# wjwei-handsome/wgatools

Hardware: AMD Instinct MI355X
Metric: paf_cigar_ops_per_s (paf2maf+stat) (higher is better)
Workload: dtype u8

## Files before the change

### wgatools_amd/csrc/capi_paf2maf.inc

```
static inline u32 job_tiles_for(int param, u64 nt) {
  if (param >= 1) return param > (int)WGA_S_MAX_JOB_TILES ? WGA_S_MAX_JOB_TILES : (u32)param;
  return nt < 200000ull ? 4u : 8u;
}

struct PrepassWs {
  u64 nt, jobs;
  u32 job_tiles;
  size_t rec_bytes, desc_bytes, list_bytes, flag_bytes, skip_bytes, zero_bytes, total;
  wga_rec_desc* recs = nullptr;
  wga_tile_desc* tdesc = nullptr;
  u32 *wide_list = nullptr, *fast_list = nullptr, *counts = nullptr;
  u8* tile_flag = nullptr;
  u32* job_skip = nullptr;
  PrepassWs(u32 n, u64 nt_, u32 job_tiles_, bool stream) : nt(nt_), jobs((nt_ + job_tiles_ - 1) / job_tiles_), job_tiles(job_tiles_) {
    rec_bytes = ((size_t)n * sizeof(wga_rec_desc) + 255) & ~(size_t)255;
    desc_bytes = (size_t)nt * sizeof(wga_tile_desc);
    list_bytes = 2 * (size_t)nt * sizeof(u32);
    flag_bytes = stream ? (((size_t)nt + 255) & ~(size_t)255) : 0;
    skip_bytes = stream ? (((size_t)jobs * sizeof(u32) + 255) & ~(size_t)255) : 0;
    zero_bytes = 256 + flag_bytes + skip_bytes;
    total = rec_bytes + desc_bytes + list_bytes + zero_bytes;
  }
  void carve(void* base) {
    char* const p = (char*)base;
    recs = (wga_rec_desc*)p;
    tdesc = (wga_tile_desc*)(p + rec_bytes);
    wide_list = (u32*)(p + rec_bytes + desc_bytes);
    fast_list = wide_list + nt;
    counts = (u32*)(p + rec_bytes + desc_bytes + list_bytes);
    tile_flag = flag_bytes ? (u8*)counts + 256 : nullptr;
    job_skip = flag_bytes ? (u32*)(tile_flag + flag_bytes) : nullptr;
  }
};
static int launch_tile_base(wga_ctx* c, const wga_cigar_batch* b, const PrepassWs& w, const wga_tile_sum* tiles, int mode,
                            int force_slow) {
  WGA_LAUNCH(k_tile_base, (u32)((w.nt + 255) / 256), WGA_BLOCK, c->stream, (const u64*)b->d_op_off, (u64)b->n_ops, tiles,
             (const wga_rec_desc*)w.recs, w.tdesc, mode, (const u8*)w.tile_flag, w.job_tiles, force_slow, w.job_skip, w.counts,
             w.fast_list, w.wide_list);
  LAUNCH_CHECK();
  return WGA_OK;
}

extern "C" {

size_t wga_tile_ws_bytes(uint64_t n_ops) { return (size_t)(n_tiles(n_ops) * sizeof(wga_tile_sum)) + 16; }

int wga_cigar_stat(wga_ctx* c, const wga_cigar_batch* b, wga_cigar_counts* d_counts,
                   wga_rec_diag* d_diag, void* d_tile_ws) {
  int rc = ctx_bind(c);
  if (rc) return rc;
  if ((rc = check_batch(b))) return rc;
  if (b->n == 0) return WGA_OK;
  if (!d_counts || !d_diag) return fail(WGA_E_INVALID_ARG, "d_counts / d_diag null", nullptr);
  RT_CHECK(rt_memset(d_counts, 0, (size_t)b->n * sizeof(wga_cigar_counts), c->stream));
  RT_CHECK(rt_memset(d_diag, 0xFF, (size_t)b->n * sizeof(wga_rec_diag), c->stream));
  u64 nt = n_tiles(b->n_ops);
  if (nt == 0) return WGA_OK;
  void* ws;
  if ((rc = ctx_scratch(c, (size_t)nt * sizeof(wga_tile_rec), &ws))) return rc;
  wga_tile_rec* tile_rec = (wga_tile_rec*)ws;
  WGA_LAUNCH(k_tile_rec, (u32)((nt + 255) / 256), WGA_BLOCK, c->stream, (const u64*)b->d_op_off,
             b->d_strand_neg, b->n, (u64)b->n_ops, tile_rec);
  LAUNCH_CHECK();
  const u32 grid = (u32)((nt + 3) / 4);
  WGA_LAUNCH(k_cigar_stat, grid, WGA_BLOCK, c->stream, b->d_ops, (const u64*)b->d_op_off,
             b->d_strand_neg, b->n, (u64)b->n_ops, (const wga_tile_rec*)tile_rec, d_counts, d_diag,
             (wga_tile_sum*)d_tile_ws);
  LAUNCH_CHECK();
  return WGA_OK;
}

int wga_exclusive_scan_u64(wga_ctx* c, uint32_t n, const uint64_t* d_in, uint64_t* d_out) {
  int rc = ctx_bind(c);
  if (rc) return rc;
  if (!d_out || (n && !d_in)) return fail(WGA_E_INVALID_ARG, "null array", nullptr);
  ScanPlain f;
  f.in = (const u64*)d_in;
  return run_scan(c, f, n, (u64*)d_out);
}

int wga_paf2maf_layout(wga_ctx* c, uint32_t n, const wga_cigar_counts* d_counts,
                       const uint64_t* d_t_src_len, const uint64_t* d_q_src_len,
                       const uint32_t* d_pre_t, const uint32_t* d_pre_q, const uint32_t* d_post,
                       uint64_t* d_t_row_off, uint64_t* d_q_row_off, uint64_t* d_rec_off) {
  int rc = ctx_bind(c);
  if (rc) return rc;
  if (!d_rec_off) return fail(WGA_E_INVALID_ARG, "d_rec_off null", nullptr);
  if (n && (!d_counts || !d_t_src_len || !d_q_src_len || !d_t_row_off || !d_q_row_off))
    return fail(WGA_E_INVALID_ARG, "null array", nullptr);
  ScanLayout f;
  f.counts = d_counts;
  f.t_src_len = (const u64*)d_t_src_len;
  f.q_src_len = (const u64*)d_q_src_len;
  f.pre_t = d_pre_t;
  f.pre_q = d_pre_q;
  f.post = d_post;
  rc = run_scan(c, f, n, (u64*)d_rec_off);
  if (rc) return rc;
  if (n) {
    WGA_LAUNCH(k_layout_rows, (n + 255u) / 256u, WGA_BLOCK, c->stream, f, n, (const u64*)d_rec_off,
               (u64*)d_t_row_off, (u64*)d_q_row_off);
    LAUNCH_CHECK();
  }
  return WGA_OK;
}

int wga_paf2maf_expand(wga_ctx* c, const wga_cigar_batch* b, const wga_cigar_counts* d_counts,
                       const void* d_tile_ws, const uint8_t* d_t_fa, uint64_t t_fa_bytes,
                       const uint64_t* d_t_src_off, const uint64_t* d_t_src_len,
                       const uint8_t* d_q_fa, uint64_t q_fa_bytes, const uint64_t* d_q_src_off,
                       const uint64_t* d_q_src_len, uint8_t* d_out, const uint64_t* d_t_row_off,
                       const uint64_t* d_q_row_off, wga_rec_diag* d_diag) {
  int rc = ctx_bind(c);
  if (rc) return rc;
  if ((rc = check_batch(b))) return rc;
  if (b->n == 0 || b->n_ops == 0) return WGA_OK;
  if (!d_counts || !d_tile_ws || !d_t_src_off || !d_t_src_len || !d_q_src_off || !d_q_src_len ||
      !d_out || !d_t_row_off || !d_q_row_off || !d_diag)
    return fail(WGA_E_INVALID_ARG, "null array", nullptr);
  if ((t_fa_bytes && !d_t_fa) || (q_fa_bytes && !d_q_fa)) return fail(WGA_E_INVALID_ARG, "null sequence pool", nullptr);
  u64 nt = n_tiles(b->n_ops);
  if (nt > 0x7FFFFFFFull) return fail(WGA_E_INVALID_ARG, "batch too large for one launch", nullptr);
  const int variant = c->expand_variant >= 0 ? c->expand_variant : WGA_AUTO_LONG_VARIANT;
  c->expand_variant_used = variant;
  const bool stream = variant == 3;
  PrepassWs w(b->n, nt, job_tiles_for(c->expand_job_tiles, nt), stream);
  void* ws;
  if ((rc = ctx_scratch(c, w.total, &ws))) return rc;
  w.carve(ws);
  if (stream) RT_CHECK(rt_memset(w.counts, 0, w.zero_bytes, c->stream));
  WGA_LAUNCH(k_rec_desc, (b->n + 255u) / 256u, WGA_BLOCK, c->stream, b->n, d_counts,
             b->d_strand_neg, (const u64*)d_t_src_off, (const u64*)d_t_src_len,
             (const u64*)d_q_src_off, (const u64*)d_q_src_len, (const u64*)d_t_row_off,
             (const u64*)d_q_row_off, w.recs, (const u64*)b->d_op_off, (u64)t_fa_bytes, (u64)q_fa_bytes, w.tile_flag);
  LAUNCH_CHECK();
  if ((rc = launch_tile_base(c, b, w, (const wga_tile_sum*)d_tile_ws, 0, c->expand_force_slow))) return rc;
  if (stream) c->stream_counts = w.counts;
  ExpandArgs a;
  a.ops = b->d_ops;
  a.op_off = (const u64*)b->d_op_off;
  a.n_ops = b->n_ops;
  a.tdesc = w.tdesc;
  a.recs = w.recs;
  a.t_fa = d_t_fa;
  a.t_fa_bytes = t_fa_bytes;
  a.q_fa = d_q_fa;
  a.q_fa_bytes = q_fa_bytes;
  a.out = d_out;
  a.diag = d_diag;
  a.force_slow = c->expand_force_slow;
  a.no_table = c->expand_no_table;
  a.drain_min = c->expand_drain_min ? c->expand_drain_min : ((u64)t_fa_bytes + (u64)q_fa_bytes > WGA_DRAIN_POOL_BYTES ? 16u : 32u);
  a.tile_count = nullptr;
  a.tile_list = nullptr;
  a.n_rec = b->n;
  a.job_tiles = w.job_tiles;
  a.job_skip = w.job_skip;
  c->expand_drain_min_used = a.drain_min;
  const uint32_t slot = c->ev_n % (uint32_t)wga_ctx::kTimingRing;
  if (c->timing) RT_CHECK(rt_event_record(c->ev[2 * slot], c->stream));
  if (stream) {
    WGA_LAUNCH(k_paf2maf_expand_s, (u32)w.jobs, 128u, c->stream, a);
    LAUNCH_CHECK();
    const u32 side_grid = nt < 256 ? (u32)nt : 256u;
    a.tile_count = w.counts;
    a.tile_list = w.fast_list;
    WGA_LAUNCH(k_paf2maf_expand_list, side_grid, WGA_BLOCK, c->stream, a);
    LAUNCH_CHECK();
    a.force_slow = 1;
    a.tile_count = w.counts + 1;
    a.tile_list = w.wide_list;
    WGA_LAUNCH(k_paf2maf_expand_list, side_grid, WGA_BLOCK, c->stream, a);
    LAUNCH_CHECK();
  } else {
    WGA_LAUNCH(k_paf2maf_expand, (u32)nt, WGA_BLOCK, c->stream, a);
    LAUNCH_CHECK();
  }
  if (c->timing) {
    RT_CHECK(rt_event_record(c->ev[2 * slot + 1], c->stream));
    c->ev_n++;
  }
  return WGA_OK;
}

int wga_ctx_expand_timing(wga_ctx* c, double* ms_sum, uint32_t* launches) {
  int rc = ctx_bind(c);
  if (rc) return rc;
  if (!ms_sum || !launches) return fail(WGA_E_INVALID_ARG, "null argument", nullptr);
  *ms_sum = 0.0;
  *launches = 0;
  if (!c->timing) return WGA_OK;
  const uint32_t n = c->ev_n < (uint32_t)wga_ctx::kTimingRing ? c->ev_n : (uint32_t)wga_ctx::kTimingRing;
  for (uint32_t k = 0; k < n; k++) {
    float ms = 0.0f;
    RT_CHECK(rt_event_elapsed_ms(c->ev[2 * k], c->ev[2 * k + 1], &ms));
    *ms_sum += (double)ms;
  }
  *launches = n;
  c->ev_n = 0;
  return WGA_OK;
}

int wga_scatter_bytes(wga_ctx* c, uint32_t n, const uint8_t* d_src, const uint64_t* d_src_off,
                      uint8_t* d_dst, const uint64_t* d_dst_off) {
  int rc = ctx_bind(c);
  if (rc) return rc;
  if (n == 0) return WGA_OK;
  if (!d_src || !d_src_off || !d_dst || !d_dst_off) return fail(WGA_E_INVALID_ARG, "null array", nullptr);
  WGA_LAUNCH(k_scatter_bytes, (n + 3u) / 4u, WGA_BLOCK, c->stream, n, d_src, (const u64*)d_src_off,
             d_dst, (const u64*)d_dst_off);
  LAUNCH_CHECK();
  return WGA_OK;
}

int wga_counts_total(wga_ctx* c, uint32_t n, const wga_cigar_counts* d_counts, uint64_t* d_totals) {
  int rc = ctx_bind(c);
  if (rc) return rc;
  if (!d_totals || (n && !d_counts)) return fail(WGA_E_INVALID_ARG, "null array", nullptr);
  static_assert(sizeof(wga_cigar_counts) == 88, "wga_cigar_counts is 11 u64");
  RT_CHECK(rt_memset(d_totals, 0, 88, c->stream));
  if (n == 0) return WGA_OK;
  u32 grid = (u32)(((u64)n * 11ull + 253ull * 8ull - 1ull) / (253ull * 8ull));
  if (grid > 2048u) grid = 2048u;
  WGA_LAUNCH(k_counts_total, grid, WGA_BLOCK, c->stream, n, (const u64*)d_counts, (u64*)d_totals);
  LAUNCH_CHECK();
  return WGA_OK;
}

}
```

### wgatools_amd/csrc/wga_capi.cpp

```cpp
#include <stdio.h>
#include <stdlib.h>
#include <string.h>

#include <algorithm>
#include <string>
#include <utility>
#include <vector>

#include <type_traits>

#include "wga_kernels.h"
#include "wga_k1_stat.h"
#include "wga_scan.h"
#include "wga_k2_v1.h"
#include "wga_kernels_k2s.h"
#include "wga_k_class.h"
#include "wga_k_peers.h"
#include "wga_k5_pafcov.h"
#include "wga_k6_pafpseudo.h"
#include "wga_k3_maf.h"
#include "wga_k7_paf_call.h"
#include "wga_k8_tokenise.h"
#include "wga_text_out.h"
#include "wga_chain_items.h"
#include "wga_paf_head.h"
#include "wga_k9_bed.h"
#include "wga_k10_chain.h"
#include "wga_k11_bridges.h"
#include "wga_k12_dotplot.h"
#include "wga_k13_splitters.h"
#include "wga_k15_fasta.h"
#include "wga_k18_bgzf_deflate.h"
#include "wga_k16_paf_call_vcf.h"
#include "wga_k17_bgzf_inflate.h"
#include "wga_k19_maf_call.h"
#include "wga_k20_maf_chunk.h"
#include "wga_k21_maf_slice.h"
#include "wga_k22_maf_rewrite.h"
#include "wga_k23_chain_split.h"
#include "wga_k24_paf_filter.h"
#include "wga_k25_chain_write.h"
#include "wga_k26_dotplot_csv.h"
#include "wga_k27_chain2paf.h"
#include "wga_k28_maf2paf.h"
#include "wga_k29_paf_fix.h"
#include "wga_k30_chain_heads.h"
#include "wga_k31_pseudo_frame.h"
#include "wga_k32_maf_frame.h"
#include "wga_k33_stat_rows.h"

struct DevBuf {
  void* mem = nullptr;
  size_t cap = 0;
  int reserve(wga_ctx* c, size_t need, size_t grow, bool* grew = nullptr);
  void release() {
    if (mem) (void)rt_free(mem);
    mem = nullptr, cap = 0;
  }
};

struct CallKey {
  int who = 0;
  struct Arr {
    const void* p = nullptr;
    size_t bytes = 0;
  } arr[5];
  uint64_t par[6] = {0, 0, 0, 0, 0, 0};
  bool operator==(const CallKey& o) const {
    bool same = who == o.who;
    for (int k = 0; k < 5; k++) same = same && arr[k].p == o.arr[k].p && arr[k].bytes == o.arr[k].bytes;
    for (int k = 0; k < 6; k++) same = same && par[k] == o.par[k];
    return same;
  }
};
struct CallCache {
  CallKey key;
  bool valid = false;
  bool take(const CallKey& k, bool is_fill) {
    const bool hit = is_fill && valid && key == k;
    valid = false;
    return hit;
  }
  void keep(const CallKey& k) { key = k, valid = true; }
  void written(const void* lo, size_t bytes) {
    const uintptr_t a = (uintptr_t)lo, z = a + (bytes ? bytes : 1);
    for (const CallKey::Arr& q : key.arr)
      if (q.p && (uintptr_t)q.p < z && (uintptr_t)q.p + (q.bytes ? q.bytes : 1) > a) valid = false;
  }
};

struct wga_ctx {
  int device = 0;
  wga_stream_t own_stream = nullptr;
  wga_stream_t stream = nullptr;
  int expand_force_slow = 0;
  int expand_no_table = 0;
  unsigned expand_drain_min = 0;
  unsigned expand_drain_min_used = 0;
  uint64_t op_long_ops = 16384;
  uint64_t op_piece_ops = 8192;
  uint64_t maf_long_cols = 32768;
  uint64_t maf_piece_cols = 16384;
  unsigned paf_pair_hash_bits = 64;
  unsigned maf_group = 0;
  DevBuf maf_tab;
  bool maf_hdr_clean = false;
  CallCache maf_cache;
  int expand_variant = -1;
  int expand_variant_used = 0;
  int expand_job_tiles = 0;
  int pseudo_variant = 3;
  const u32* pseudo_counts = nullptr;
  const u32* stream_counts = nullptr;
  DevBuf scratch;
  struct OpTab {
    DevBuf buf;
    CallCache cache;
    uint32_t np = 0;
    bool all = false;
    u64* piece_off = nullptr;
    u32* piece_rec = nullptr;
    void* pieces = nullptr;
  } op_tab;
  struct ClassTab {
    DevBuf buf;
    CallCache cache;
    wga_tile_sum* tiles = nullptr;
    wga_class_sums* rec_sums = nullptr;
  } class_tab;
  struct ElemScan {
    DevBuf buf;
    CallCache cache;
  } elem_scan;
  struct Cov {
    DevBuf pieces;
    DevBuf tile_list;
    DevBuf order;
    std::vector<u64> order_key;
    DevBuf list;
    u64 list_rcap = 0;
  } cov;
  bool rs_have_ev = false;
  rt_event_t rs_ready, rs_done;
  std::vector<wga_stream_t> rs_streams;
  std::vector<rt_event_t> rs_copied;
  bool rs_same_device_ok = false;
  bool rs_staged = false;
#ifdef WGA_EMU
  u32 cov_spin_limit = 64;
#else
  u32 cov_spin_limit = 1u << 12;
#endif
  static const int kTimingRing = 64;
  bool timing = false;
  rt_event_t ev[2 * kTimingRing];
  uint32_t ev_n = 0;
};

static thread_local std::string g_last_error;

static int fail(int code, const char* what, const char* detail) {
  g_last_error = std::string(what) + (detail ? std::string(": ") + detail : std::string());
  return code;
}
#define RT_CHECK(expr)                                      \
  do {                                                      \
    const char* _e = (expr);                                \
    if (_e) return fail(WGA_E_HIP, #expr, _e);              \
  } while (0)
#define LAUNCH_CHECK()                                      \
  do {                                                      \
    const char* _e = rt_launch_error();                     \
    if (_e) return fail(WGA_E_HIP, "kernel launch", _e);    \
  } while (0)

static int ctx_bind(wga_ctx* c) {
  if (!c) return fail(WGA_E_INVALID_ARG, "null context", nullptr);
  RT_CHECK(rt_set_device(c->device));
  return WGA_OK;
// ... 96 lines not shown
  wga_ctx* c = new wga_ctx();
  c->device = device;
  const char* e = rt_set_device(device);
  if (!e) e = rt_stream_create(&c->own_stream);
  if (e) {
    delete c;
    return fail(WGA_E_HIP, "context creation", e);
  }
  c->stream = c->own_stream;
  if (const char* v = getenv("WGA_EXPAND_VARIANT")) c->expand_variant = (atoi(v) == 0 || atoi(v) == 3) ? atoi(v) : -1;
  if (const char* v = getenv("WGA_EXPAND_DRAIN_MIN")) {
    const int d = atoi(v);
    if (d >= 0 && d <= 64) c->expand_drain_min = (unsigned)d;
  }
  *out = c;
  return WGA_OK;
}

void wga_ctx_destroy(wga_ctx* c) {
  if (!c) return;
  (void)rt_set_device(c->device);
  (void)rt_sync(c->stream);
  if (c->timing)
    for (int k = 0; k < 2 * wga_ctx::kTimingRing; k++) rt_event_destroy(c->ev[k]);
  if (c->rs_have_ev) rt_event_destroy(c->rs_ready), rt_event_destroy(c->rs_done);
  for (rt_event_t e : c->rs_copied) rt_event_destroy(e);
  for (wga_stream_t st : c->rs_streams) rt_stream_destroy(st);
  for (DevBuf* b : {&c->scratch, &c->maf_tab, &c->op_tab.buf, &c->class_tab.buf, &c->elem_scan.buf, &c->cov.pieces,
                    &c->cov.tile_list, &c->cov.order, &c->cov.list})
    b->release();
  rt_stream_destroy(c->own_stream);
  delete c;
}

int wga_ctx_set_stream(wga_ctx* c, void* hip_stream) {
  int rc = ctx_bind(c);
  if (rc) return rc;
#ifdef WGA_EMU
  (void)hip_stream;
  return WGA_OK;
#else
  if (c->stream != (wga_stream_t)hip_stream) RT_CHECK(rt_sync(c->stream));
  c->stream = (wga_stream_t)hip_stream;
  return WGA_OK;
#endif
}

int wga_ctx_reset_stream(wga_ctx* c) {
  int rc = ctx_bind(c);
  if (rc) return rc;
  if (c->stream != c->own_stream) RT_CHECK(rt_sync(c->stream));
  c->stream = c->own_stream;
  return WGA_OK;
}

int wga_ctx_set_param(wga_ctx* c, const char* name, int64_t value) {
  if (!c || !name) return fail(WGA_E_INVALID_ARG, "null argument", nullptr);
  if (strcmp(name, "expand_force_slow") == 0) {
    c->expand_force_slow = value != 0;
    return WGA_OK;
  }
  if (strcmp(name, "reduce_same_device_ok") == 0) {
    c->rs_same_device_ok = value != 0;
    return WGA_OK;
  }
  if (strcmp(name, "cov_spin_limit") == 0) {
    if (value < 0 || value > 0x7FFFFFFF) return fail(WGA_E_INVALID_ARG, "cov_spin_limit: 0 .. 2^31 - 1", nullptr);
    c->cov_spin_limit = (u32)value;
    return WGA_OK;
  }
  if (strcmp(name, "reduce_staged") == 0) {
    c->rs_staged = value != 0;
    return WGA_OK;
  }
  if (strcmp(name, "expand_drain_min") == 0) {
    if (value < 0 || value > 64) return fail(WGA_E_INVALID_ARG, "expand_drain_min: 0 .. 64", nullptr);
    c->expand_drain_min = (unsigned)value;
    return WGA_OK;
  }
  if (strcmp(name, "expand_no_table") == 0) {
    c->expand_no_table = value != 0;
    return WGA_OK;
  }
  if (strcmp(name, "op_long_ops") == 0) {
    if (value < 1) return fail(WGA_E_INVALID_ARG, "must be positive", name);
    c->op_long_ops = (uint64_t)value;
    return WGA_OK;
  }
  if (strcmp(name, "op_piece_ops") == 0) {
    if (value < 256 || (value & 255)) return fail(WGA_E_INVALID_ARG, "a positive multiple of 256", name);
    c->op_piece_ops = (uint64_t)value;
    return WGA_OK;
  }
  if (strcmp(name, "maf_long_cols") == 0 || strcmp(name, "maf_piece_cols") == 0) {
    if (value < 1) return fail(WGA_E_INVALID_ARG, "must be positive", name);
    (name[4] == 'l' ? c->maf_long_cols : c->maf_piece_cols) = (uint64_t)value;
    return WGA_OK;
  }
  if (strcmp(name, "maf_group") == 0) {
    if (value < 0 || value > (long long)WGA_MAF_G) return fail(WGA_E_INVALID_ARG, "maf_group: 0 (by the batch) .. 8", nullptr);
    c->maf_group = (unsigned)value;
    return WGA_OK;
  }
  if (strcmp(name, "paf_pair_hash_bits") == 0) {
    if (value < 1 || value > 64) return fail(WGA_E_INVALID_ARG, "paf_pair_hash_bits: 1 .. 64", nullptr);
    c->paf_pair_hash_bits = (unsigned)value;
    return WGA_OK;
  }
  if (strcmp(name, "expand_variant") == 0) {
    if (value != -1 && value != 0 && value != 3) return fail(WGA_E_INVALID_ARG, "expand_variant: -1 (the library's choice), 0, 3", nullptr);
    c->expand_variant = (int)value;
    return WGA_OK;
  }
  if (strcmp(name, "expand_job_tiles") == 0) {
    if (value < 0 || value > (int64_t)WGA_S_MAX_JOB_TILES) return fail(WGA_E_INVALID_ARG, "expand_job_tiles: 0 (by the batch), 1 .. 32", nullptr);
    c->expand_job_tiles = (int)value;
    return WGA_OK;
  }
  if (strcmp(name, "pseudo_variant") == 0) {
    if (value != 0 && value != 3) return fail(WGA_E_INVALID_ARG, "pseudo_variant: 0, 3", nullptr);
    c->pseudo_variant = (int)value;
    return WGA_OK;
  }
  if (strcmp(name, "expand_timing") == 0) {
    if (value && !c->timing) {
      int rc = ctx_bind(c);
      if (rc) return rc;
      for (int k = 0; k < 2 * wga_ctx::kTimingRing; k++) {
        const char* e = rt_event_create(&c->ev[k]);
        if (e) {
          for (int j = 0; j < k; j++) rt_event_destroy(c->ev[j]);
          return fail(WGA_E_HIP, "rt_event_create", e);
        }
      }
    }
    if (!value && c->timing)
      for (int k = 0; k < 2 * wga_ctx::kTimingRing; k++) rt_event_destroy(c->ev[k]);
    c->timing = value != 0;
    c->ev_n = 0;
    return WGA_OK;
  }
  return fail(WGA_E_INVALID_ARG, "unknown parameter", name);
}

int wga_sync(wga_ctx* c) {
  int rc = ctx_bind(c);
  if (rc) return rc;
  RT_CHECK(rt_sync(c->stream));
  return WGA_OK;
}
int wga_malloc(wga_ctx* c, size_t bytes, void** d_out) {
  int rc = ctx_bind(c);
  if (rc) return rc;
  if (!d_out) return fail(WGA_E_INVALID_ARG, "d_out is null", nullptr);
  const char* e = rt_malloc(d_out, bytes);
  if (e) return fail(WGA_E_OOM, "device allocation", e);
  return WGA_OK;
}
static void ctx_arrays_written(wga_ctx* c, const void* lo, size_t bytes) {
  for (CallCache* k : {&c->maf_cache, &c->op_tab.cache, &c->elem_scan.cache, &c->class_tab.cache}) k->written(lo, bytes);
}

int wga_free(wga_ctx* c, void* d_ptr) {
  int rc = ctx_bind(c);
  if (rc) return rc;
  if (d_ptr) ctx_arrays_written(c, d_ptr, 0);
// ... 125 lines not shown
```

### wgatools_amd/csrc/wga_intrin.h

```cpp
#ifndef WGA_INTRIN_H
#define WGA_INTRIN_H

#ifdef WGA_EMU
#include "wga_intrin_emu.h"
#else

#define WGA_UNI32(x) ((u32)__builtin_amdgcn_readfirstlane((int)(x)))
#define WGA_UNI64(x)                                                               \
  (((u64)(u32)__builtin_amdgcn_readfirstlane((int)((u64)(x) >> 32)) << 32) |       \
   (u64)(u32)__builtin_amdgcn_readfirstlane((int)(u32)(u64)(x)))

#define WGA_WAVE_ID(t) ((u32)__builtin_amdgcn_readfirstlane((int)((u32)(t) >> 6)))

#define WGA_PIN(x) asm volatile("" : "+v"(x))
#define WGA_PIN4(a, b, c, d) asm volatile("" : "+v"(a), "+v"(b), "+v"(c), "+v"(d))
#define WGA_PIN7(a, b, c, d, e, f, g) asm volatile("" : "+v"(a), "+v"(b), "+v"(c), "+v"(d), "+v"(e), "+v"(f), "+v"(g))

__device__ __forceinline__ u32 wave_incl_scan_u32(u32 v) {
  v += (u32)__builtin_amdgcn_update_dpp(0, (int)v, 0x111, 0xF, 0xF, false);
  v += (u32)__builtin_amdgcn_update_dpp(0, (int)v, 0x112, 0xF, 0xF, false);
  v += (u32)__builtin_amdgcn_update_dpp(0, (int)v, 0x114, 0xF, 0xF, false);
  v += (u32)__builtin_amdgcn_update_dpp(0, (int)v, 0x118, 0xF, 0xF, false);
  v += (u32)__builtin_amdgcn_update_dpp(0, (int)v, 0x142, 0xA, 0xF, false);
  v += (u32)__builtin_amdgcn_update_dpp(0, (int)v, 0x143, 0xC, 0xF, false);
// ... 53 lines not shown
#define WGA_STREAM_AUX 2
#endif
__device__ __forceinline__ void buf_store16_stream(const BufRsrc& r, u32 off, const u32 v[4]) {
  const u32x4_v x = {v[0], v[1], v[2], v[3]};
  __builtin_amdgcn_raw_buffer_store_b128(x, r, (int)off, 0, WGA_STREAM_AUX);
}

__device__ __forceinline__ u64 wave_get_u64(u32 v, int k) {
  return (u64)(u32)__builtin_amdgcn_readlane((int)v, k) | ((u64)(u32)__builtin_amdgcn_readlane((int)v, k + 1) << 32);
}
__device__ __forceinline__ u32 wave_get_u32(u32 v, int k) { return (u32)__builtin_amdgcn_readlane((int)v, k); }
__device__ __forceinline__ u32 wave_get_u32_dyn(u32 v, u32 k) { return (u32)__builtin_amdgcn_readlane((int)v, (int)k); }
#define WGA_CLOCK() ((u64)__builtin_amdgcn_s_memtime())
#define WGA_SLEEP(n) __builtin_amdgcn_s_sleep(n)
#define WGA_WAVE_SYNC() __builtin_amdgcn_wave_barrier()

__device__ __forceinline__ u32 lane_rank(u64 m, u32 lane) {
  (void)lane;
  return (u32)__builtin_amdgcn_mbcnt_hi((u32)(m >> 32), __builtin_amdgcn_mbcnt_lo((u32)m, 0u));
}

__device__ __forceinline__ u32x4_a16 ops_load16(const u32* p) {
  return *(const u32x4_a16*)p;
}

__device__ __forceinline__ u32 bit_mask(u32 bits, u32 idx) { return (u32)__builtin_amdgcn_sbfe((int)bits, idx, 1u); }
__device__ __forceinline__ u32 bit_test(u32 bits, u32 idx) { return __builtin_amdgcn_ubfe(bits, idx, 1u); }

#define WGA_KARG_SPACE __attribute__((address_space(4)))
#define WGA_KARG_SEGMENT(T, a) ((T)__builtin_amdgcn_kernarg_segment_ptr())
#define WGA_KARG_FRESH(p) asm volatile("" : "+s"(p))

#ifndef WGA_W_STORE_AUX
#define WGA_W_STORE_AUX 2
#endif
__device__ __forceinline__ void buf_store16_w(const BufRsrc& r, u32 off, const u32 v[4]) {
  const u32x4_v x = {v[0], v[1], v[2], v[3]};
  __builtin_amdgcn_raw_buffer_store_b128(x, r, (int)off, 0, WGA_W_STORE_AUX);
}

__device__ __forceinline__ void lds_dma16(const void* gbase, u32 voff, void* lds_dst) {
  const u64 gb = WGA_UNI64((u64)gbase);
  const u32 ld = WGA_UNI32((u32)(u64)lds_dst);
  u32 keep;
  asm volatile("s_mov_b32 %0, m0\n\ts_mov_b32 m0, %3\n\ts_nop 0\n\tglobal_load_lds_dwordx4 %1, %2\n\ts_mov_b32 m0, %0"
               : "=&s"(keep)
               : "v"(voff), "s"(gb), "s"(ld)
               : "memory");
}
__device__ __forceinline__ void lds_dma16_after_reads(const void* gbase, u32 voff, void* lds_dst) {
  asm volatile("s_waitcnt lgkmcnt(0)" ::: "memory");
  lds_dma16(gbase, voff, lds_dst);
}
__device__ __forceinline__ void gstore16_nt(void* base, u32 voff, const u32 v[4]) {
  const u64 b = WGA_UNI64((u64)base);
  const u32x4_v x = {v[0], v[1], v[2], v[3]};
  asm volatile("global_store_dwordx4 %0, %1, %2 nt" ::"v"(voff), "v"(x), "s"(b) : "memory");
}
__device__ __forceinline__ void vm_wait(u32 k) {
  switch (k) {
    case 0: asm volatile("s_waitcnt vmcnt(0)" ::: "memory"); break;
    case 1: asm volatile("s_waitcnt vmcnt(1)" ::: "memory"); break;
    case 2: asm volatile("s_waitcnt vmcnt(2)" ::: "memory"); break;
    case 3: asm volatile("s_waitcnt vmcnt(3)" ::: "memory"); break;
    case 4: asm volatile("s_waitcnt vmcnt(4)" ::: "memory"); break;
    case 5: asm volatile("s_waitcnt vmcnt(5)" ::: "memory"); break;
    case 6: asm volatile("s_waitcnt vmcnt(6)" ::: "memory"); break;
    case 7: asm volatile("s_waitcnt vmcnt(7)" ::: "memory"); break;
    case 8: asm volatile("s_waitcnt vmcnt(8)" ::: "memory"); break;
    case 9: asm volatile("s_waitcnt vmcnt(9)" ::: "memory"); break;
    case 10: asm volatile("s_waitcnt vmcnt(10)" ::: "memory"); break;
    case 11: asm volatile("s_waitcnt vmcnt(11)" ::: "memory"); break;
    case 12: asm volatile("s_waitcnt vmcnt(12)" ::: "memory"); break;
    case 13: asm volatile("s_waitcnt vmcnt(13)" ::: "memory"); break;
    case 14: asm volatile("s_waitcnt vmcnt(14)" ::: "memory"); break;
    case 15: asm volatile("s_waitcnt vmcnt(15)" ::: "memory"); break;
    default: asm volatile("" ::: "memory"); break;
  }
}
__device__ __forceinline__ u32 bfi_b32(u32 mask, u32 a, u32 b) { return (a & mask) | (b & ~mask); }

#endif

struct wga_u64x2 {
  u64 x, y;
};
#if defined(__HIP_DEVICE_COMPILE__) && !defined(WGA_EMU)
#define WGA_RO_SPACE __attribute__((address_space(4)))
#define WGA_RO32(p) (*(const WGA_RO_SPACE u32*)(u64)(const u32*)(p))
#define WGA_RO64(p) (*(const WGA_RO_SPACE u64*)(u64)(const u64*)(p))
__device__ __forceinline__ wga_u64x2 wga_ro16(const u64* p) {
  typedef u64 u64x2_v __attribute__((vector_size(16)));
  const u64x2_v v = *(const WGA_RO_SPACE u64x2_v*)(u64)p;
  return {v[0], v[1]};
}
#define WGA_RO_HERE2(a, b) asm volatile("" ::"s"(a), "s"(b))
#define WGA_RO_HERE4(a, b, c, d) asm volatile("" ::"s"(a), "s"(b), "s"(c), "s"(d))
#define WGA_VM_LANDED() __builtin_amdgcn_s_waitcnt(0x0F70)
#define WGA_VM_LEFT6() __builtin_amdgcn_s_waitcnt(0x0F76)
#else
#define WGA_RO32(p) (*(const u32*)(p))
#define WGA_RO64(p) (*(const u64*)(p))
__device__ __forceinline__ wga_u64x2 wga_ro16(const u64* p) { return {p[0], p[1]}; }
#define WGA_RO_HERE2(a, b) ((void)0)
#define WGA_RO_HERE4(a, b, c, d) ((void)0)
#define WGA_VM_LANDED() ((void)0)
#define WGA_VM_LEFT6() ((void)0)
#endif
#if defined(__HIP_DEVICE_COMPILE__) && !defined(WGA_EMU)
#define WGA_GLOBAL_STORE_U8(p, v) (*(__attribute__((address_space(1))) u8*)(p) = (v))
#else
#define WGA_GLOBAL_STORE_U8(p, v) (*(u8*)(p) = (v))
#endif

#endif
```

### wgatools_amd/csrc/wga_k1_stat.h

```cpp
#ifndef WGA_K1_STAT_H
#define WGA_K1_STAT_H

#include "wga_kernels.h"

#ifndef WGA_K1_BLOCKS
#define WGA_K1_BLOCKS 5
#endif

struct wga_tile_rec {
  u32 rec, neg;
  u64 rs, re;
};
__global__ __launch_bounds__(256) void k_tile_rec(const u64* __restrict__ op_off,
                                                  const u8* __restrict__ strand_neg, u32 n, u64 n_ops,
                                                  wga_tile_rec* __restrict__ tile_rec) {
  const u64 g = (u64)blockIdx.x * 256 + threadIdx.x;
  const u64 x = g * WGA_TILE;
  if (x >= n_ops) return;
  u32 lo = 0, hi = n;
  while (hi - lo > 1u) {
    const u32 mid = lo + ((hi - lo) >> 1);
    if (op_off[mid] <= x)
      lo = mid;
    else
      hi = mid;
  }
  wga_tile_rec t;
  t.rec = lo;
  t.neg = strand_neg[lo] != 0 ? 1u : 0u;
  t.rs = op_off[lo];
  t.re = op_off[lo + 1];
  tile_rec[g] = t;
}

__device__ __forceinline__ void cigar_stat_tile(const u64 g, const u32 (&w)[16], const u32 lane, const u64* __restrict__ op_off,
                                                const u8* __restrict__ strand_neg, u64 n_ops,
                                                const wga_tile_rec* __restrict__ tile_rec, wga_cigar_counts* counts,
                                                wga_rec_diag* diag, wga_tile_sum* tiles) {
  const u64 tile_start = g * WGA_TILE;
  const u64 tile_end = tile_start + WGA_TILE < n_ops ? tile_start + WGA_TILE : n_ops;

  const wga_tile_rec tr = tile_rec[g];
  u32 r = WGA_UNI32(tr.rec);
  const u32 r_first = r;
  u64 cur = tile_start;
  u64 tot[5] = {0, 0, 0, 0, 0}, tail[5] = {0, 0, 0, 0, 0};
  u64 re = WGA_UNI64(tr.re);
  constexpr u32 MX_BITS = 0x01810181u, I_BITS = 0x02020202u, X_BITS = 0x01000100u, RARE_BITS = 0xF878F878u;
  constexpr u32 IEV_BITS = 0x00020002u, DEV_BITS = 0x00040004u;
  const u32 lane4 = lane * 4u;
  auto wave_sums = [&](u32 s_mx, u32 s_i, u32 s_t, u32 s_x, u32 ev, u64& Smx, u64& Si, u64& St, u64& Sx, u32& EV) {
    if (__ballot(s_t >= (1u << 26)) == 0ull) {
      Smx = wave_sum_u32(s_mx), Si = wave_sum_u32(s_i), St = wave_sum_u32(s_t), Sx = wave_sum_u32(s_x);
    } else {
      Smx = wave_sum_u32_wide(s_mx), Si = wave_sum_u32_wide(s_i), St = wave_sum_u32_wide(s_t), Sx = wave_sum_u32_wide(s_x);
    }
    EV = wave_sum_u32(ev);
  };
  u64 Wmx, Wi, Wt, Wx;
  u32 Wev;
  bool rare_tile;
  {
    u32 s_mx = 0, s_i = 0, s_t = 0, s_x = 0, ev = 0, rare = 0;
#pragma unroll
    for (int k = 0; k < 16; k++) {
      const u32 op = w[k], len = op >> 4;
      s_mx += len & bit_mask(MX_BITS, op);
      s_i += len & bit_mask(I_BITS, op);
      s_t += len;
      s_x += len & bit_mask(X_BITS, op);
      ev += bit_test(IEV_BITS, op);
      ev += bit_test(DEV_BITS, op) << 16;
      rare |= bit_mask(RARE_BITS, op);
    }
    rare_tile = __ballot(rare != 0u) != 0ull;
    wave_sums(s_mx, s_i, s_t, s_x, ev, Wmx, Wi, Wt, Wx, Wev);
  }
  u64 Amx = 0, Ai = 0, At = 0, Ax = 0;
  u32 Aev = 0;
  while (cur < tile_end) {
    while (re <= cur) {
      r++;
      re = op_off[r + 1];
    }
    const bool first = r == r_first;
    const u64 rs = first ? WGA_UNI64(tr.rs) : op_off[r];
    const bool neg = first ? (WGA_UNI32(tr.neg) != 0u) : (strand_neg[r] != 0);
    const u64 seg_end = re < tile_end ? re : tile_end;
    const u32 a = (u32)(cur - tile_start), b = (u32)(seg_end - tile_start);

    u64 S[5], Sx, St;
    u32 EV, BAD = 0xFFFFFFFFu;
    S[3] = S[4] = 0ull;
    if (!rare_tile && seg_end == tile_end) {
      S[0] = Wmx - Amx, S[1] = Wi - Ai, St = Wt - At, Sx = Wx - Ax;
      EV = Wev - Aev;
    } else {
      const u32 span = b - a;
      u32 s_mx = 0, s_i = 0, s_t = 0, s_s = 0, s_o = 0;
      u32 s_x = 0;
      u32 ev = 0;
      u32 bad = 0xFFFFFFFFu;
      u32 rare = 0;
#pragma unroll
      for (int k = 0; k < 16; k++) {
        const u32 idx = (u32)(k >> 2) * 256u + (u32)(k & 3) + lane4;
        const u32 op = (idx - a < span) ? w[k] : 0u;
        const u32 len = op >> 4;
        s_mx += len & bit_mask(MX_BITS, op);
        s_i += len & bit_mask(I_BITS, op);
        s_t += len;
        s_x += len & bit_mask(X_BITS, op);
        ev += bit_test(IEV_BITS, op);
        ev += bit_test(DEV_BITS, op) << 16;
        rare |= bit_mask(RARE_BITS, op);
      }
      const bool any_rare = rare_tile && __ballot(rare != 0u) != 0ull;
      if (any_rare) {
#pragma unroll
        for (int k = 0; k < 16; k++) {
          const u32 idx = (u32)(k >> 2) * 256u + (u32)(k & 3) + lane4;
          u32 op = (idx - a < span) ? w[k] : 0u;
          WGA_PIN(op);
          const u32 cls = op_class(op & 15u), len = op >> 4;
          s_s += cls == CLS_S ? len : 0u;
          s_o += cls == CLS_O ? len : 0u;
          bad = (cls >= CLS_S && idx < bad) ? idx : bad;
        }
      }
      wave_sums(s_mx, s_i, s_t, s_x, ev, S[0], S[1], St, Sx, EV);
      if (any_rare) {
        S[3] = wave_sum_u32_wide(s_s);
        S[4] = wave_sum_u32_wide(s_o);
        BAD = wave_min_u32(bad);
      }
      Amx += S[0], Ai += S[1], At += St, Ax += Sx, Aev += EV;
    }
    S[2] = St - S[0] - S[1] - S[3] - S[4];
    const u64 Smatch = S[0] - Sx;

    {
      const bool whole = rs >= tile_start && re <= tile_end;
      const u64 match = Smatch, mism = S[0] - Smatch;
      const u64 iev = EV & 0xFFFFu, dev = EV >> 16;
      const u64 z = 0;
      u64 v = 0;
      v = lane_put_u64<0u>(v, match, lane);
      v = lane_put_u64<1u>(v, mism, lane);
      v = lane_put_u64<2u>(v, neg ? z : iev, lane);
      v = lane_put_u64<3u>(v, neg ? z : S[1], lane);
      v = lane_put_u64<4u>(v, neg ? z : dev, lane);
      v = lane_put_u64<5u>(v, neg ? z : S[2], lane);
      v = lane_put_u64<6u>(v, neg ? iev : z, lane);
      v = lane_put_u64<7u>(v, neg ? S[1] : z, lane);
      v = lane_put_u64<8u>(v, neg ? dev : z, lane);
      v = lane_put_u64<9u>(v, neg ? S[2] : z, lane);
// ... 72 lines not shown
```

### wgatools_amd/csrc/wga_k2_v1.h

```cpp
#ifndef WGA_K2_V1_H
#define WGA_K2_V1_H

#include "wga_kernels.h"

#ifndef WGA_DRAIN_MIN
#define WGA_DRAIN_MIN 32u
#endif
#ifndef WGA_DRAIN_POOL_BYTES
#define WGA_DRAIN_POOL_BYTES (192ull << 20)
#endif
struct RowSrc {
  const u8* fa;
  u64 fa_bytes;
  u64 src_off;
  u64 src_len;
  bool rc;
  bool safe;
  u32 drain_min = WGA_DRAIN_MIN;
  const u8* win_base;
};

struct WinRaw {
  u32 v[4];
};
// ... 714 lines not shown
    for (int job = 0; job < 4; job++) {
      const bool is_q = (job & 1) != 0, is_tail = job >= 2;
      if (is_tail && (!rec_ends || !(rec_flags & (is_q ? 4u : 2u)))) continue;
#ifndef WGA_OWN_STRIDE
#define WGA_OWN_STRIDE 2u
#endif
      const u32 own0 = ((u32)job * (WGA_OWN_STRIDE == 2u ? 1u : 2u) + nseg) & 3u, own1 = (own0 + WGA_OWN_STRIDE) & 3u;
      if (!is_tail && seg_cols <= WGA_SOLO_BYTES && own0 != wave && own1 != wave) continue;
      const int q2 = is_q ? 2 : 0, q4 = is_q ? 4 : 0;
      const u64 gap_total = wave_get_u64(dsc, 26 + q2);
      const u64 L = wave_get_u64(dsc, 30);
      const u64 src_len = is_q ? q_src_len : t_src_len;
      const u64 row_len = src_len + gap_total;
      u64 x0, nbytes;
      if (!is_tail) {
        if (!fast) continue;
        const u64 x1 = cb + seg_cols < row_len ? cb + seg_cols : row_len;
        x0 = cb;
        nbytes = x1 > cb ? x1 - cb : 0;
      } else {
        if (!rec_ends) continue;
        x0 = L;
        nbytes = row_len > L ? row_len - L : 0;
      }
      if (nbytes == 0) continue;
      const bool coop = nbytes > WGA_SOLO_BYTES;
      const u32 c_row = is_tail ? 0u : col_a;
      u64 cut = nbytes;
      if (!coop && nbytes > WGA_SPLIT_BYTES) {
        const u32 cc = (c_row + (u32)(nbytes >> 1)) & ~15u;
        if (cc > c_row && (u64)(cc - c_row) < nbytes) cut = cc - c_row;
      }
      for (int piece = 0; piece < 2; piece++) {
        const u64 lo = piece == 0 ? 0 : cut, hi = piece == 0 ? cut : nbytes;
        if (lo >= hi) continue;
        if (!coop && (piece == 0 ? own0 : own1) != wave) continue;
        RowSrc src;
        src.fa = is_q ? a.q_fa : a.t_fa;
        src.fa_bytes = is_q ? a.q_fa_bytes : a.t_fa_bytes;
        src.src_off = wave_get_u64(dsc, 18 + q4);
        src.src_len = src_len;
        src.rc = is_q && (wave_get_u32(dsc, 3) & 1u) != 0u;
        src.drain_min = a.drain_min;
        u8* const dst = a.out + wave_get_u64(dsc, 14 + q2) + x0;
        const u64 sb0 = is_tail ? L - gap_total : (is_q ? qb : tb);
        for (u64 done = lo; done < hi; done += (1ull << 30)) {
          const u64 m = hi - done < (1ull << 30) ? hi - done : (1ull << 30);
          RowDesc rd;
          rd.c_org = is_tail ? 0u : col_a;
          rd.G_col = is_q ? s_qg_col : s_tg_col;
          rd.G_cum = is_q ? s_qg_cum : s_tg_cum;
          rd.G_adj = is_tail ? s_zero2 : rd.G_cum;
          rd.ga = is_tail ? 0 : (is_q ? ja : ia);
          rd.gb = is_tail ? 0 : (is_q ? jb : ib);
          rd.gcum_a = is_tail ? 0u : (is_q ? dcum_a : icum_a);
          rd.sbase = is_tail ? sb0 + done : sb0;
          rd.lowmask = s_lowmask;
          rd.tbl = is_tail ? s_zero2 : s_tbl;
          rd.tsh = (is_q && !is_tail) ? 16u : 0u;
          rd.gsh = is_tail ? 31u : gsh;
          rd.queue = s_queue;
          rowsrc_prepare(src, rd.sbase);
          emit_row(dst + done, (u32)m, is_tail ? 0u : col_a + (u32)done, rd, src, coop ? tid : lane,
                   coop ? WGA_BLOCK : 64u, bad_base);
        }
      }
    }
    cur = seg_end;
    r++;
    if (cur < tile_end) re = a.op_off[r + 1];
    nseg++;
  }
}

__device__ __forceinline__ u64 xcd_tile_of_block() {
  const u32 nt = gridDim.x, b = blockIdx.x, x = b & 7u, q = nt >> 3, r = nt & 7u;
  return (u64)(x * q + (x < r ? x : r) + (b >> 3));
}
__global__ __launch_bounds__(256, WGA_K2_BLOCKS) void k_paf2maf_expand(ExpandArgs a) {
  expand_tile_v1(a, xcd_tile_of_block());
}

__global__ __launch_bounds__(256, 4) void k_paf2maf_expand_list(ExpandArgs a) {
  const u32 n_list = *a.tile_count;
  for (u32 idx = blockIdx.x; idx < n_list; idx += gridDim.x) {
    expand_tile_v1(a, a.tile_list[idx]);
    __syncthreads();
  }
}

#endif
```

### wgatools_amd/csrc/wga_kernels.h

```cpp
#ifndef WGA_KERNELS_H
#define WGA_KERNELS_H

#include "../../include/wga_hip.h"
#include "wga_rt.h"

typedef unsigned int u32;
typedef unsigned long long u64;
typedef long long i64;
typedef unsigned char u8;

#define WGA_TILE 1024u
#define WGA_BLOCK 256u
#define WGA_FAST_COL_LIMIT 0x7FFFFFFFull

#define CLS_MX 0u
#define CLS_I 1u
#define CLS_D 2u
#define CLS_S 3u
#define CLS_O 4u

__device__ __forceinline__ u32 op_class(u32 code) {
  const u64 lut = (u64)CLS_MX | ((u64)CLS_I << 3) | ((u64)CLS_D << 6) | ((u64)CLS_O << 9) |
                  ((u64)CLS_S << 12) | ((u64)CLS_O << 15) | ((u64)CLS_O << 18) |
                  ((u64)CLS_MX << 21) | ((u64)CLS_MX << 24) | ((u64)CLS_I << 27) |
// ... 125 lines not shown
__global__ __launch_bounds__(256) void k_layout_rows(ScanLayout f, u32 n, const u64* rec_off,
                                                     u64* t_row_off, u64* q_row_off) {
  u32 i = blockIdx.x * 256u + threadIdx.x;
  if (i >= n) return;
  u64 t = rec_off[i] + (f.pre_t ? f.pre_t[i] : 0u);
  u64 q = t + f.t_row(i) + (f.pre_q ? f.pre_q[i] : 0u);
  t_row_off[i] = t;
  q_row_off[i] = q;
}

__device__ __forceinline__ u32 comp4(u32 x, u32* bad) {
  const u32 sel = x & 0x07070707u;
  const u32 fold = byte_perm(0x474EFF54u, 0x43FF41FFu, sel);
  const u32 comp = byte_perm(0x434EFF41u, 0x47FF54FFu, sel);
  *bad = (x & 0xDFDFDFDFu) ^ fold;
  return comp | (x & 0x20202020u);
}

__device__ __forceinline__ u32 bswap32(u32 x) {
  return (x >> 24) | ((x >> 8) & 0xFF00u) | ((x << 8) & 0xFF0000u) | (x << 24);
}
__device__ __forceinline__ u32 alignbyte(u32 hi, u32 lo, u32 sh) {
  return (u32)(((((u64)hi) << 32) | (u64)lo) >> (8u * sh));
}
__device__ __forceinline__ u32 bytemask(int lo, int hi) {
  lo = lo < 0 ? 0 : lo;
  hi = hi > 4 ? 4 : hi;
  if (hi <= lo) return 0u;
  u32 mh = hi >= 4 ? 0xFFFFFFFFu : ((1u << (8 * hi)) - 1u);
  u32 ml = (1u << (8 * lo)) - 1u;
  return mh & ~ml;
}

struct wga_rec_desc {
  u64 t_row_off, q_row_off;
  u64 t_src_off, t_src_len, q_src_off, q_src_len;
  u64 I_total, D_total, L;
  u64 neg;
};
struct wga_tile_base {
  u64 mx, i, d;
};
struct wga_tile_desc {
  u64 tile_cols;
  u32 rec, neg;
  u64 b_mx, b_i, b_d;
  u64 rs, re;
  u64 t_row_off, q_row_off, t_src_off, t_src_len, q_src_off, q_src_len, I_total, D_total, L;
};

__global__ __launch_bounds__(256) void k_rec_desc(u32 n, const wga_cigar_counts* counts,
                                                  const u8* strand_neg, const u64* t_src_off,
                                                  const u64* t_src_len, const u64* q_src_off,
                                                  const u64* q_src_len, const u64* t_row_off,
                                                  const u64* q_row_off, wga_rec_desc* out, const u64* op_off,
                                                  u64 t_fa_bytes, u64 q_fa_bytes, u8* tile_flag) {
  u32 r = blockIdx.x * 256u + threadIdx.x;
  if (r >= n) return;
  const wga_cigar_counts cn = counts[r];
  wga_rec_desc d;
  d.t_row_off = t_row_off[r];
  d.q_row_off = q_row_off[r];
  d.t_src_off = t_src_off[r];
  d.t_src_len = t_src_len[r];
  d.q_src_off = q_src_off[r];
  d.q_src_len = q_src_len[r];
  d.I_total = cn.ins_bp + cn.inv_ins_bp;
  d.D_total = cn.del_bp + cn.inv_del_bp;
  d.L = cn.match + cn.mismatch + d.I_total + d.D_total;
  d.neg = (strand_neg[r] != 0 ? 1u : 0u) | (d.t_src_len + d.I_total > d.L ? 2u : 0u) | (d.q_src_len + d.D_total > d.L ? 4u : 0u) |
          ((d.t_src_len + d.I_total < d.L || d.q_src_len + d.D_total < d.L) ? 8u : 0u);
  out[r] = d;
  if (!tile_flag) return;
  const bool inside = d.t_src_off >= 32ull && d.t_src_off + d.t_src_len + 32ull <= t_fa_bytes && d.q_src_off >= 32ull &&
                      d.q_src_off + d.q_src_len + 32ull <= q_fa_bytes;
  if ((d.neg & 0xEull) == 0ull && inside) return;
  const u64 a = op_off[r], b = op_off[r + 1];
  if (b <= a) return;
  for (u64 t = a / WGA_TILE; t <= (b - 1) / WGA_TILE; t++) tile_flag[t] = 1;
}

#define WGA_S_MAX_TILE_COLS (1ull << 24)
#define WGA_S_SKIP 0x100u
__global__ __launch_bounds__(256) void k_tile_base(const u64* op_off, u64 n_ops,
                                                   const wga_tile_sum* tiles,
                                                   const wga_rec_desc* recs, wga_tile_desc* descs, int pseudo,
                                                   const u8* tile_flag, u32 job_tiles, int all_slow, u32* job_skip,
                                                   u32* counts, u32* list_fast, u32* list_slow) {
  const u32 lane = threadIdx.x & 63u;
  const u64 g = (u64)blockIdx.x * 256 + threadIdx.x;
  const u64 tile_start = g * WGA_TILE;
  const bool valid = tile_start < n_ops;
  wga_tile_sum ts;
  u64 rs = 0, re = 0, g0 = 0;
  if (valid) {
    ts = tiles[g];
    rs = op_off[ts.rec];
    re = op_off[ts.rec + 1];
  }
  u64 p_mx = 0, p_i = 0, p_d = 0;
  bool far = false;
  if (valid && rs < tile_start) {
    g0 = rs / WGA_TILE;
    if (g - g0 <= 64) {
      for (u64 k = g0; k < g; k++) {
        const u64* v = (k == g0) ? tiles[k].tail : tiles[k].tot;
        p_mx += v[CLS_MX];
        p_i += v[CLS_I] + (pseudo ? v[CLS_S] : 0ull);
        p_d += v[CLS_D];
      }
    } else {
      far = true;
    }
  }
  u64 m = __ballot(far);
  while (m) {
    const int src = (int)__builtin_ctzll(m);
    const u64 gg = __shfl(g, src), gg0 = __shfl(g0, src);
    u64 a_mx = 0, a_i = 0, a_d = 0;
    for (u64 k = gg0 + lane; k < gg; k += 64) {
      const u64* v = (k == gg0) ? tiles[k].tail : tiles[k].tot;
      a_mx += v[CLS_MX];
      a_i += v[CLS_I] + (pseudo ? v[CLS_S] : 0ull);
      a_d += v[CLS_D];
    }
    a_mx = wave_sum_u64(a_mx);
    a_i = wave_sum_u64(a_i);
    a_d = wave_sum_u64(a_d);
    if ((int)lane == src) {
      p_mx = a_mx;
      p_i = a_i;
      p_d = a_d;
    }
    m &= m - 1;
  }
  if (!valid) return;
  const wga_rec_desc rd = recs[ts.rec];
  wga_tile_desc d;
  d.tile_cols = ts.tot[CLS_MX] + ts.tot[CLS_I] + ts.tot[CLS_D] + (pseudo ? ts.tot[CLS_S] : 0ull);
  d.rec = (u32)ts.rec;
  d.neg = (u32)rd.neg;
  if (tile_flag) {
    const bool slow = all_slow || d.tile_cols > WGA_FAST_COL_LIMIT;
    if (slow || tile_flag[g] || d.tile_cols > WGA_S_MAX_TILE_COLS) {
      d.neg |= WGA_S_SKIP;
      atomicOr(&job_skip[g / job_tiles], all_slow ? 0xFFFFFFFFu : 1u << (u32)(g % job_tiles));
      if (slow)
        list_slow[atomicAdd(&counts[1], 1u)] = (u32)g;
      else
        list_fast[atomicAdd(&counts[0], 1u)] = (u32)g;
    }
  }
  d.b_mx = p_mx;
  d.b_i = p_i;
  d.b_d = p_d;
  d.rs = rs;
  d.re = re;
  d.t_row_off = rd.t_row_off;
  d.q_row_off = rd.q_row_off;
  d.t_src_off = rd.t_src_off;
  d.t_src_len = rd.t_src_len;
  d.q_src_off = rd.q_src_off;
  d.q_src_len = rd.q_src_len;
  d.I_total = rd.I_total;
  d.D_total = rd.D_total;
  d.L = rd.L;
  descs[g] = d;
}

struct ExpandArgs {
  const u32* ops;
  const u64* op_off;
  u64 n_ops;
  const wga_tile_desc* tdesc;
  const wga_rec_desc* recs;
  const u8* t_fa;
  u64 t_fa_bytes;
  const u8* q_fa;
  u64 q_fa_bytes;
  u8* out;
  wga_rec_diag* diag;
  int force_slow;
  int no_table;
  u32 drain_min;
  const u32* tile_count;
  const u32* tile_list;
  u32 n_rec;
  u32 job_tiles;
  const u32* job_skip;
};

#endif
```

Baseline: 83.47 billion.

## Fuse stat memsets into prologue, merge expand list launches, trim tile_base work

Folds the two memsets of counts and diag into the tile-record kernel, so one prologue kernel clears the outputs and builds tile records. The two expand_list launches become one that walks the fast list and then the wide list. k_tile_base now writes descriptors only for tiles that need them: skipped tiles, tiles at the start of a job, and tiles that follow a skipped tile. The cigar stat inner loop gains a fast path using 24-bit multiply-add and a seen-bitmask when no op length has its high bits set. Each change removes a launch or some memory traffic, but the descriptor trimming relies on the streaming kernel never reading the skipped descriptors, and a debug poison option is added to check that.

After: 82.48 billion. 1.2% lower.

```diff
diff --git a/wgatools_amd/csrc/capi_paf2maf.inc b/wgatools_amd/csrc/capi_paf2maf.inc
--- a/wgatools_amd/csrc/capi_paf2maf.inc
+++ b/wgatools_amd/csrc/capi_paf2maf.inc
@@ -34,6 +34,7 @@
 };
 static int launch_tile_base(wga_ctx* c, const wga_cigar_batch* b, const PrepassWs& w, const wga_tile_sum* tiles, int mode,
                             int force_slow) {
+  if (c->prepass_poison_desc) RT_CHECK(rt_memset(w.tdesc, 0xFF, w.desc_bytes, c->stream));
   WGA_LAUNCH(k_tile_base, (u32)((w.nt + 255) / 256), WGA_BLOCK, c->stream, (const u64*)b->d_op_off, (u64)b->n_ops, tiles,
              (const wga_rec_desc*)w.recs, w.tdesc, mode, (const u8*)w.tile_flag, w.job_tiles, force_slow, w.job_skip, w.counts,
              w.fast_list, w.wide_list);
@@ -52,15 +53,21 @@
   if ((rc = check_batch(b))) return rc;
   if (b->n == 0) return WGA_OK;
   if (!d_counts || !d_diag) return fail(WGA_E_INVALID_ARG, "d_counts / d_diag null", nullptr);
-  RT_CHECK(rt_memset(d_counts, 0, (size_t)b->n * sizeof(wga_cigar_counts), c->stream));
-  RT_CHECK(rt_memset(d_diag, 0xFF, (size_t)b->n * sizeof(wga_rec_diag), c->stream));
   u64 nt = n_tiles(b->n_ops);
-  if (nt == 0) return WGA_OK;
+  if (nt == 0) {
+    RT_CHECK(rt_memset(d_counts, 0, (size_t)b->n * sizeof(wga_cigar_counts), c->stream));
+    RT_CHECK(rt_memset(d_diag, 0xFF, (size_t)b->n * sizeof(wga_rec_diag), c->stream));
+    return WGA_OK;
+  }
   void* ws;
   if ((rc = ctx_scratch(c, (size_t)nt * sizeof(wga_tile_rec), &ws))) return rc;
   wga_tile_rec* tile_rec = (wga_tile_rec*)ws;
-  WGA_LAUNCH(k_tile_rec, (u32)((nt + 255) / 256), WGA_BLOCK, c->stream, (const u64*)b->d_op_off,
-             b->d_strand_neg, b->n, (u64)b->n_ops, tile_rec);
+  static_assert(sizeof(wga_cigar_counts) == 88 && sizeof(wga_rec_diag) == 24, "k_stat_prologue clears 11 + 3 u64 per record");
+  const u64 words = (u64)b->n * 14ull, fill_threads = (words + 3) / 4;
+  const u64 pro_threads = nt > fill_threads ? nt : fill_threads;
+  if ((pro_threads + 255) / 256 > 0x7FFFFFFFull) return fail(WGA_E_INVALID_ARG, "batch too large for one launch", nullptr);
+  WGA_LAUNCH(k_stat_prologue, (u32)((pro_threads + 255) / 256), WGA_BLOCK, c->stream, (const u64*)b->d_op_off,
+             b->d_strand_neg, b->n, (u64)b->n_ops, tile_rec, (u64*)d_counts, (u64*)d_diag);
   LAUNCH_CHECK();
   const u32 grid = (u32)((nt + 3) / 4);
   WGA_LAUNCH(k_cigar_stat, grid, WGA_BLOCK, c->stream, b->d_ops, (const u64*)b->d_op_off,
@@ -153,6 +160,7 @@
   a.drain_min = c->expand_drain_min ? c->expand_drain_min : ((u64)t_fa_bytes + (u64)q_fa_bytes > WGA_DRAIN_POOL_BYTES ? 16u : 32u);
   a.tile_count = nullptr;
   a.tile_list = nullptr;
+  a.tile_list_wide = nullptr;
   a.n_rec = b->n;
   a.job_tiles = w.job_tiles;
   a.job_skip = w.job_skip;
@@ -165,11 +173,7 @@
     const u32 side_grid = nt < 256 ? (u32)nt : 256u;
     a.tile_count = w.counts;
     a.tile_list = w.fast_list;
-    WGA_LAUNCH(k_paf2maf_expand_list, side_grid, WGA_BLOCK, c->stream, a);
-    LAUNCH_CHECK();
-    a.force_slow = 1;
-    a.tile_count = w.counts + 1;
-    a.tile_list = w.wide_list;
+    a.tile_list_wide = w.wide_list;
     WGA_LAUNCH(k_paf2maf_expand_list, side_grid, WGA_BLOCK, c->stream, a);
     LAUNCH_CHECK();
   } else {
diff --git a/wgatools_amd/csrc/wga_capi.cpp b/wgatools_amd/csrc/wga_capi.cpp
--- a/wgatools_amd/csrc/wga_capi.cpp
+++ b/wgatools_amd/csrc/wga_capi.cpp
@@ -95,6 +95,7 @@
   wga_stream_t stream = nullptr;
   int expand_force_slow = 0;
   int expand_no_table = 0;
+  int prepass_poison_desc = 0;
   unsigned expand_drain_min = 0;
   unsigned expand_drain_min_used = 0;
   uint64_t op_long_ops = 16384;
@@ -357,6 +358,10 @@
     c->expand_no_table = value != 0;
     return WGA_OK;
   }
+  if (strcmp(name, "prepass_poison_desc") == 0) {
+    c->prepass_poison_desc = value != 0;
+    return WGA_OK;
+  }
   if (strcmp(name, "op_long_ops") == 0) {
     if (value < 1) return fail(WGA_E_INVALID_ARG, "must be positive", name);
     c->op_long_ops = (uint64_t)value;
diff --git a/wgatools_amd/csrc/wga_intrin.h b/wgatools_amd/csrc/wga_intrin.h
--- a/wgatools_amd/csrc/wga_intrin.h
+++ b/wgatools_amd/csrc/wga_intrin.h
@@ -159,6 +159,15 @@
 
 #endif
 
+#if defined(__HIP_DEVICE_COMPILE__) && !defined(WGA_EMU)
+__device__ __forceinline__ u32 mad_u24(u32 a, u32 b, u32 acc) {
+  asm("v_mad_u32_u24 %0, %1, %2, %0" : "+v"(acc) : "v"(a), "v"(b));
+  return acc;
+}
+#else
+__device__ __forceinline__ u32 mad_u24(u32 a, u32 b, u32 acc) { return acc + (a & 0xFFFFFFu) * (b & 0xFFFFFFu); }
+#endif
+
 struct wga_u64x2 {
   u64 x, y;
 };
diff --git a/wgatools_amd/csrc/wga_k1_stat.h b/wgatools_amd/csrc/wga_k1_stat.h
--- a/wgatools_amd/csrc/wga_k1_stat.h
+++ b/wgatools_amd/csrc/wga_k1_stat.h
@@ -11,10 +11,18 @@
   u32 rec, neg;
   u64 rs, re;
 };
-__global__ __launch_bounds__(256) void k_tile_rec(const u64* __restrict__ op_off,
-                                                  const u8* __restrict__ strand_neg, u32 n, u64 n_ops,
-                                                  wga_tile_rec* __restrict__ tile_rec) {
+__global__ __launch_bounds__(256) void k_stat_prologue(const u64* __restrict__ op_off,
+                                                       const u8* __restrict__ strand_neg, u32 n, u64 n_ops,
+                                                       wga_tile_rec* __restrict__ tile_rec, u64* __restrict__ counts,
+                                                       u64* __restrict__ diag) {
   const u64 g = (u64)blockIdx.x * 256 + threadIdx.x;
+  const u64 n_counts = (u64)n * 11ull, n_words = (u64)n * 14ull, stride = (u64)gridDim.x * 256ull;
+  for (u64 k = g; k < n_words; k += stride) {
+    if (k < n_counts)
+      counts[k] = 0ull;
+    else
+      diag[k - n_counts] = ~0ull;
+  }
   const u64 x = g * WGA_TILE;
   if (x >= n_ops) return;
   u32 lo = 0, hi = n;
@@ -62,16 +70,35 @@
   bool rare_tile;
   {
     u32 s_mx = 0, s_i = 0, s_t = 0, s_x = 0, ev = 0, rare = 0;
-#pragma unroll
-    for (int k = 0; k < 16; k++) {
-      const u32 op = w[k], len = op >> 4;
-      s_mx += len & bit_mask(MX_BITS, op);
-      s_i += len & bit_mask(I_BITS, op);
-      s_t += len;
-      s_x += len & bit_mask(X_BITS, op);
-      ev += bit_test(IEV_BITS, op);
-      ev += bit_test(DEV_BITS, op) << 16;
-      rare |= bit_mask(RARE_BITS, op);
+    u32 any = 0;
+#pragma unroll
+    for (int k = 0; k < 16; k++) any |= w[k];
+    if (__ballot((any >> 28) != 0u) == 0ull) {
+      u32 seen = 0;
+#pragma unroll
+      for (int k = 0; k < 16; k++) {
+        const u32 op = w[k], len = op >> 4;
+        s_mx = mad_u24(len, bit_test(MX_BITS, op), s_mx);
+        s_i = mad_u24(len, bit_test(I_BITS, op), s_i);
+        s_t += len;
+        s_x = mad_u24(len, bit_test(X_BITS, op), s_x);
+        ev += bit_test(IEV_BITS, op);
+        ev += bit_test(DEV_BITS, op) << 16;
+        seen |= 1u << (op & 31u);
+      }
+      rare = seen & RARE_BITS;
+    } else {
+#pragma unroll
+      for (int k = 0; k < 16; k++) {
+        const u32 op = w[k], len = op >> 4;
+        s_mx += len & bit_mask(MX_BITS, op);
+        s_i += len & bit_mask(I_BITS, op);
+        s_t += len;
+        s_x += len & bit_mask(X_BITS, op);
+        ev += bit_test(IEV_BITS, op);
+        ev += bit_test(DEV_BITS, op) << 16;
+        rare |= bit_mask(RARE_BITS, op);
+      }
     }
     rare_tile = __ballot(rare != 0u) != 0ull;
     wave_sums(s_mx, s_i, s_t, s_x, ev, Wmx, Wi, Wt, Wx, Wev);
diff --git a/wgatools_amd/csrc/wga_k2_v1.h b/wgatools_amd/csrc/wga_k2_v1.h
--- a/wgatools_amd/csrc/wga_k2_v1.h
+++ b/wgatools_amd/csrc/wga_k2_v1.h
@@ -820,9 +820,12 @@
 }
 
 __global__ __launch_bounds__(256, 4) void k_paf2maf_expand_list(ExpandArgs a) {
-  const u32 n_list = *a.tile_count;
-  for (u32 idx = blockIdx.x; idx < n_list; idx += gridDim.x) {
-    expand_tile_v1(a, a.tile_list[idx]);
+  const u32 n_fast = a.tile_count[0], n_wide = a.tile_count[1];
+  const int force_slow = a.force_slow;
+  for (u64 idx = blockIdx.x; idx < (u64)n_fast + n_wide; idx += gridDim.x) {
+    const bool wide = idx >= n_fast;
+    a.force_slow = wide ? 1 : force_slow;
+    expand_tile_v1(a, wide ? a.tile_list_wide[idx - n_fast] : a.tile_list[idx]);
     __syncthreads();
   }
 }
diff --git a/wgatools_amd/csrc/wga_kernels.h b/wgatools_amd/csrc/wga_kernels.h
--- a/wgatools_amd/csrc/wga_kernels.h
+++ b/wgatools_amd/csrc/wga_kernels.h
@@ -231,6 +231,10 @@
 
 #define WGA_S_MAX_TILE_COLS (1ull << 24)
 #define WGA_S_SKIP 0x100u
+__device__ __forceinline__ u64 tile_cols_of(const wga_tile_sum* tiles, u64 g, int pseudo) {
+  const u64* const tot = tiles[g].tot;
+  return tot[CLS_MX] + tot[CLS_I] + tot[CLS_D] + (pseudo ? tot[CLS_S] : 0ull);
+}
 __global__ __launch_bounds__(256) void k_tile_base(const u64* op_off, u64 n_ops,
                                                    const wga_tile_sum* tiles,
                                                    const wga_rec_desc* recs, wga_tile_desc* descs, int pseudo,
@@ -240,16 +244,26 @@
   const u64 g = (u64)blockIdx.x * 256 + threadIdx.x;
   const u64 tile_start = g * WGA_TILE;
   const bool valid = tile_start < n_ops;
-  wga_tile_sum ts;
+  u64 tile_cols = 0, rec = 0;
+  bool left = false;
+  bool need = valid;
+  if (valid) {
+    tile_cols = tile_cols_of(tiles, g, pseudo);
+    if (tile_flag) {
+      left = all_slow || tile_flag[g] || tile_cols > WGA_S_MAX_TILE_COLS;
+      need = left || g % job_tiles == 0;
+      if (!need) need = tile_flag[g - 1] || tile_cols_of(tiles, g - 1, pseudo) > WGA_S_MAX_TILE_COLS;
+    }
+  }
   u64 rs = 0, re = 0, g0 = 0;
-  if (valid) {
-    ts = tiles[g];
-    rs = op_off[ts.rec];
-    re = op_off[ts.rec + 1];
+  if (need) {
+    rec = tiles[g].rec;
+    rs = op_off[rec];
+    re = op_off[rec + 1];
   }
   u64 p_mx = 0, p_i = 0, p_d = 0;
   bool far = false;
-  if (valid && rs < tile_start) {
+  if (need && rs < tile_start) {
     g0 = rs / WGA_TILE;
     if (g - g0 <= 64) {
       for (u64 k = g0; k < g; k++) {
@@ -283,22 +297,20 @@
     }
     m &= m - 1;
   }
-  if (!valid) return;
-  const wga_rec_desc rd = recs[ts.rec];
+  if (!need) return;
+  const wga_rec_desc rd = recs[rec];
   wga_tile_desc d;
-  d.tile_cols = ts.tot[CLS_MX] + ts.tot[CLS_I] + ts.tot[CLS_D] + (pseudo ? ts.tot[CLS_S] : 0ull);
-  d.rec = (u32)ts.rec;
+  d.tile_cols = tile_cols;
+  d.rec = (u32)rec;
   d.neg = (u32)rd.neg;
-  if (tile_flag) {
-    const bool slow = all_slow || d.tile_cols > WGA_FAST_COL_LIMIT;
-    if (slow || tile_flag[g] || d.tile_cols > WGA_S_MAX_TILE_COLS) {
-      d.neg |= WGA_S_SKIP;
-      atomicOr(&job_skip[g / job_tiles], all_slow ? 0xFFFFFFFFu : 1u << (u32)(g % job_tiles));
-      if (slow)
-        list_slow[atomicAdd(&counts[1], 1u)] = (u32)g;
-      else
-        list_fast[atomicAdd(&counts[0], 1u)] = (u32)g;
-    }
+  if (left) {
+    const bool slow = all_slow || tile_cols > WGA_FAST_COL_LIMIT;
+    d.neg |= WGA_S_SKIP;
+    atomicOr(&job_skip[g / job_tiles], all_slow ? 0xFFFFFFFFu : 1u << (u32)(g % job_tiles));
+    if (slow)
+      list_slow[atomicAdd(&counts[1], 1u)] = (u32)g;
+    else
+      list_fast[atomicAdd(&counts[0], 1u)] = (u32)g;
   }
   d.b_mx = p_mx;
   d.b_i = p_i;
@@ -337,6 +349,7 @@
   u32 n_rec;
   u32 job_tiles;
   const u32* job_skip;
+  const u32* tile_list_wide;
 };
 
 #endif
```
